# oswsnqc/Tensorflow-DPPO

Measured on AMD Instinct MI355X. Metric: env-steps/sec (whole node), Humanoid-shaped MLP DPPO at 1/2/4/8 MI355X, higher is better.
Workload: dtype fp32; 1 GPU; model=Humanoid-v4 MLP 64x64 tanh, preset=humanoid, global_batch=16777216, num_envs_per_gpu=262144, rollout_T=64, update_steps=4, parallelism=dp1

## Files before the change

dppo_amd/ops/hip/bindings.cpp:

```cpp
#include <torch/extension.h>

#include <vector>

std::vector<torch::Tensor> gae_scan(torch::Tensor rewards, torch::Tensor values,
                                    torch::Tensor dones, torch::Tensor boot,
                                    double gamma, double lam, bool whiten,
                                    double eps, torch::Tensor adv_out,
                                    torch::Tensor etr_out);

torch::Tensor ppo_loss_gauss_fwd(torch::Tensor pdpi, torch::Tensor pdold,
                                 torch::Tensor vpred, torch::Tensor oldv,
                                 torch::Tensor act, torch::Tensor adv,
                                 torch::Tensor etr, double clip,
                                 double entcoeff, double vcoeff);

torch::Tensor ppo_loss_gauss_gh(torch::Tensor pdflat, torch::Tensor oldflat,
                                torch::Tensor vpred, torch::Tensor oldv,
                                torch::Tensor act, torch::Tensor adv,
                                torch::Tensor etr, double clip,
                                double entcoeff, double vcoeff,
                                torch::Tensor clip_dev);

std::vector<torch::Tensor> ppo_loss_gauss_bwd(
    torch::Tensor pdpi, torch::Tensor pdold, torch::Tensor vpred,
    torch::Tensor oldv, torch::Tensor act, torch::Tensor adv,
    torch::Tensor etr, double clip, double entcoeff, double vcoeff,
    torch::Tensor gtotal);

torch::Tensor ppo_loss_cat_fwd(torch::Tensor lpi, torch::Tensor lold,
                               torch::Tensor vpred, torch::Tensor oldv,
                               torch::Tensor act, torch::Tensor adv,
                               torch::Tensor etr, double clip,
                               double entcoeff, double vcoeff);

std::vector<torch::Tensor> ppo_loss_cat_bwd(
    torch::Tensor lpi, torch::Tensor lold, torch::Tensor vpred,
    torch::Tensor oldv, torch::Tensor act, torch::Tensor adv,
    torch::Tensor etr, double clip, double entcoeff, double vcoeff,
    torch::Tensor gtotal);

torch::Tensor cat_sample(torch::Tensor logits, int64_t seed, int64_t ctr);

void bf16_mm256(torch::Tensor A, torch::Tensor B, torch::Tensor C,
                int64_t epi, torch::Tensor bias, torch::Tensor aux,
                torch::Tensor grad, int64_t grad_off, torch::Tensor CT,
                int64_t ldt, torch::Tensor sums, int64_t sums_off);

void bf16_mm_small(torch::Tensor A, torch::Tensor B, torch::Tensor C,
                   torch::Tensor C2, torch::Tensor aux, torch::Tensor grad,
                   int64_t g1_off, int64_t g2_off, int64_t srow, int64_t epi,
                   int64_t m_real, int64_t n_real, int64_t ldc,
                   torch::Tensor bias);

void bf16_transpose(torch::Tensor in, torch::Tensor out, torch::Tensor sums,
                    int64_t sums_off, int64_t R, int64_t C, int64_t ld_in,
                    int64_t ld_out);

void gauss_gh_wide(torch::Tensor pdflat_bf, torch::Tensor oldflat,
                   torch::Tensor v_bf, torch::Tensor oldv, torch::Tensor act,
                   torch::Tensor adv, torch::Tensor etr, torch::Tensor gh,
                   torch::Tensor clip_dev, double clip, double entcoeff,
                   double vcoeff);

void adam_step(torch::Tensor p, torch::Tensor g, torch::Tensor m,
               torch::Tensor v, int64_t step, double lr, double beta1,
               double beta2, double eps);

void adam_step_dev(torch::Tensor p, torch::Tensor g, torch::Tensor m,
                   torch::Tensor v, torch::Tensor step_dev,
                   torch::Tensor lr_dev, torch::Tensor coef, double beta1,
                   double beta2, double eps);

void gemm_fwd(torch::Tensor X, torch::Tensor Wt, torch::Tensor bias,
              int64_t activation, int64_t heads, torch::Tensor C,
              torch::Tensor v, torch::Tensor aux, int64_t wt_layout,
              int64_t ablate, int64_t ldc);

void dw_mfma(torch::Tensor delta, torch::Tensor acts, torch::Tensor grad_buf,
             int64_t w_off, int64_t b_off, int64_t split_row, int64_t w_off2,
             int64_t b_off2, int64_t ablate);

void rollout_sample(torch::Tensor pdflat, torch::Tensor actions,
                    torch::Tensor xva, torch::Tensor seed_dev,
                    torch::Tensor eps_dev, int64_t step, int64_t va_off,
                    double act_low, double act_high);

void gemm_env_step(torch::Tensor xva, torch::Tensor M, torch::Tensor xin,
                   torch::Tensor xout, torch::Tensor envd,
                   torch::Tensor horizons, torch::Tensor t,
                   torch::Tensor epr,
                   torch::Tensor rewards, torch::Tensor dones,
                   torch::Tensor rsum, torch::Tensor seed_dev, double sigma,
                   int64_t step, torch::Tensor V, torch::Tensor xvp);

void rollout_env_step(torch::Tensor xin, torch::Tensor xout, torch::Tensor G,
                      torch::Tensor envd, torch::Tensor horizons,
                      torch::Tensor t, torch::Tensor epr,
                      torch::Tensor rewards, torch::Tensor dones,
                      torch::Tensor seed_dev, double sigma, int64_t step);

torch::Tensor rollout_moments(torch::Tensor rewards, torch::Tensor dones,
                              torch::Tensor epr_in, int64_t T, int64_t E);

bool mlp_chunk_supported(int64_t D, int64_t H, int64_t A, int64_t n_hidden);

void mlp_chunk_train(
    torch::Tensor params, torch::Tensor states, torch::Tensor actions,
    torch::Tensor adv, torch::Tensor etr, torch::Tensor oldflat,
    torch::Tensor oldv, std::vector<int64_t> offsets,
    std::vector<int64_t> dims, int64_t activation, torch::Tensor clip_dev,
    double clip, double entcoeff, double vcoeff, torch::Tensor slabs,
    torch::Tensor mom, torch::Tensor vel, torch::Tensor step_dev,
    torch::Tensor lr_dev, torch::Tensor coef, torch::Tensor flat_grad,
    bool fuse_adam, double beta1, double beta2, double eps);

bool mlp_mid_supported(int64_t H1, int64_t H2, int64_t A, int64_t n_hidden);

void mlp_mid_bwd(torch::Tensor params, std::vector<int64_t> offsets,
                 torch::Tensor h1, torch::Tensor h2, torch::Tensor pdflat,
                 torch::Tensor v, torch::Tensor oldflat, torch::Tensor oldv,
                 torch::Tensor act, torch::Tensor adv, torch::Tensor etr,
                 int64_t activation, torch::Tensor clip_dev, double clip,
                 double entcoeff, double vcoeff, torch::Tensor dz1,
                 torch::Tensor grad);

std::vector<torch::Tensor> rollout_run(
    torch::Tensor params, std::vector<int64_t> offsets,
    std::vector<int64_t> dims, int64_t activation,
    torch::Tensor envblob, int64_t rank, torch::Tensor horizons,
// ... 4 lines not shown

std::vector<torch::Tensor> rollout_run_cat(
    torch::Tensor params, std::vector<int64_t> offsets,
    std::vector<int64_t> dims, int64_t activation,
    torch::Tensor envblob, int64_t rank, torch::Tensor horizons,
    double noise, double eps_explore,
    torch::Tensor x, torch::Tensor t, torch::Tensor epr,
    int64_t T, int64_t n_actions, int64_t seed, torch::Tensor out_buf,
    int64_t ablate);

PYBIND11_MODULE(TORCH_EXTENSION_NAME, mod) {
  mod.def("gae_scan", &gae_scan,
          "segmented GAE reverse scan + whitening (gfx950)");
  mod.def("ppo_loss_gauss_fwd", &ppo_loss_gauss_fwd,
          "fused DiagGaussian PPO loss forward (gfx950)");
  mod.def("ppo_loss_gauss_bwd", &ppo_loss_gauss_bwd,
          "fused DiagGaussian PPO loss backward (gfx950)");
  mod.def("ppo_loss_cat_fwd", &ppo_loss_cat_fwd,
          "fused Categorical PPO loss forward (gfx950)");
  mod.def("ppo_loss_cat_bwd", &ppo_loss_cat_bwd,
          "fused Categorical PPO loss backward (gfx950)");
  mod.def("cat_sample", &cat_sample,
          "Gumbel-max categorical sampling, counter-based RNG (gfx950)");
  mod.def("bf16_mm256", &bf16_mm256,
          "bf16 MFMA GEMM, 256^2 tile, pipelined glds, fused epilogues "
          "(gfx950)");
  mod.def("bf16_mm_small", &bf16_mm_small,
          "guarded bf16 MFMA GEMM for ragged heads shapes (gfx950)");
  mod.def("bf16_transpose", &bf16_transpose,
          "bf16 2D transpose with fused column sums (gfx950)");
  mod.def("gauss_gh_wide", &gauss_gh_wide,
          "wide-policy PPO loss gradient -> bf16 [g_pd | g_v] (gfx950)");
  mod.def("adam_step", &adam_step, "fused flat Adam step (gfx950)");
  mod.def("adam_step_dev", &adam_step_dev,
          "graph-replayable fused Adam (device step/lr) (gfx950)");
  mod.def("rollout_run", &rollout_run,
          "fused T-step rollout: MLP fwd + sample + synthetic env (gfx950)");
  mod.def("rollout_run_cat", &rollout_run_cat,
          "fused T-step rollout, Discrete/Categorical policy: MLP fwd + "
          "Gumbel-max sample + synthetic env, int64 actions (gfx950)");
  mod.def("rollout_sample", &rollout_sample,
          "per-step action sampling + eps-greedy (v3 rollout) (gfx950)");
  mod.def("gemm_env_step", &gemm_env_step,
          "fused G-GEMM + env transition epilogue + per-env finish, "
          "optionally folding the next step's x@V (v3 rollout; gfx950)");
  mod.def("rollout_env_step", &rollout_env_step,
          "per-step synthetic env finish: tanh/reward/done/reset (gfx950)");
  mod.def("rollout_moments", &rollout_moments,
          "episode-reward moments from reward/done streams (gfx950)");
  mod.def("ppo_loss_gauss_gh", &ppo_loss_gauss_gh,
          "wave-per-row PPO loss gradient -> [g_pd | g_v] (gfx950)");
  mod.def("gemm_fwd", &gemm_fwd,
          "MFMA f32 layer forward C=act(X@Wt+b), fused tanh (gfx950)");
  mod.def("dw_mfma", &dw_mfma,
          "MFMA f32 split-K dW += delta^T@acts into flat grad (gfx950)");
  mod.def("mlp_chunk_supported", &mlp_chunk_supported,
          "shape eligibility for the fused chunk-step kernel (gfx950)");
  mod.def("mlp_chunk_train", &mlp_chunk_train,
          "fused small-MLP training chunk step: fwd+PPO grad+bwd+dW "
          "partials + slab-reduce Adam (gfx950)");
  mod.def("mlp_mid_supported", &mlp_mid_supported,
          "shape eligibility for the fused update-middle kernel (gfx950)");
  mod.def("mlp_mid_bwd", &mlp_mid_bwd,
          "fused update middle: PPO grad + heads/L2 dgrad + dW2/heads dW "
          "partials -> dz1 and flat grad, no gh/dz2 in HBM (gfx950)");
}
```

dppo_amd/ops/hip/mfma_gemm.hip:

```cpp

#include <hip/hip_runtime.h>
#include <torch/extension.h>
#include <c10/hip/HIPStream.h>

#include "common.h"

namespace {

using f32x16 = __attribute__((ext_vector_type(16))) float;
using f32x4 = __attribute__((ext_vector_type(4))) float;

constexpr int BK = 16;
constexpr int M_WAVE = 32;
constexpr int FWD_WAVES = 4;
constexpr int FWD_M = FWD_WAVES * M_WAVE;
constexpr int MAX_NT = 4;

DEV_INLINE int cd_row(int reg, int lane) {
  return (reg & 3) + 8 * (reg >> 2) + 4 * (lane >> 5);
}


struct FwdArgs {
  const float* X;
// ... 300 lines not shown
        issue_w(kb + PBK);
      }
      __syncthreads();

      const int ksteps = min(PBK, a.K - kb);
      #pragma unroll 4
      for (int k2 = 0; k2 < ksteps; k2 += 2) {
        const float av = xs[wave * M_WAVE + i_l][k2 + k_l];
        #pragma unroll
        for (int t = 0; t < NT; ++t) {
          const float bv = ws[k2 + k_l][t * M_WAVE + i_l];
          acc[t] = __builtin_amdgcn_mfma_f32_32x32x2f32(av, bv, acc[t], 0, 0, 0);
        }
      }
      __syncthreads();
    }

    #pragma unroll
    for (int t = 0; t < NT; ++t) {
      const int col = n0 + t * M_WAVE + i_l;
      if (col < a.N) {
        const float bv = (a.activation >= 3) ? 0.f : a.bias[col];
        #pragma unroll
        for (int r = 0; r < 16; ++r) {
          const int64_t row = b0 + wave * M_WAVE + cd_row(r, lane);
          if (row < a.B) {
            float x;
            if (a.activation >= 3) {
              const float h = a.aux[row * a.N + col];
              x = acc[t][r] * ((a.activation == 3) ? (1.f - h * h)
                                                   : (h > 0.f ? 1.f : 0.f));
            } else {
              x = acc[t][r] + bv;
              if (a.activation == 0) x = fmaxf(x, 0.f);
              else if (a.activation == 1) x = fast_tanhf(x);
            }
            if (a.heads == 2) {
              if (col == a.N - 2) a.v[row] = x;
              else if (col < a.N - 2) a.C[row * a.ldc + col] = x;
            } else if (a.heads) {
              if (col == a.N - 1) a.v[row] = x;
              else a.C[row * a.ldc + col] = x;
            } else {
              a.C[row * a.ldc + col] = x;
            }
          }
        }
      }
    }
  }
}


template <int RING,
          bool ENV = false>
__launch_bounds__(FWD_WAVES * 64, RING == 2 ? 6 : RING == 3 ? 4 : 3)
__global__ void gemm_fwd_glds_kernel(FwdArgs a) {
  constexpr int NT = 2;
  constexpr int PBK = 16;
  constexpr int NW = NT * M_WAVE;
  constexpr int XB = FWD_M * PBK * 4;
  constexpr int WB = PBK * NW * 4;
  constexpr int SLOT = XB + WB;
  __shared__ __attribute__((aligned(16))) char smem[RING * SLOT];
  const int tid = threadIdx.x;
  const int lane = tid & (WAVE - 1);
  const int wave = tid / WAVE;
  const int i_l = lane & 31;
  const int k_l = lane >> 5;
  const int n0 = blockIdx.y * NW;

  const int64_t b0 = (int64_t)blockIdx.x * FWD_M;
  if (b0 >= a.B) return;

  const float* srcX[2];
  int xcol[2];
  int64_t xrow[2];
  #pragma unroll
  for (int p = 0; p < 2; ++p) {
    const int q = tid + p * FWD_WAVES * 64;
    const int r = q >> 2;
    const int c4 = (q & 3) ^ (r & 3);
    int64_t row = b0 + r;
    row = row < a.B ? row : a.B - 1;
    xrow[p] = row;
    xcol[p] = c4 * 4;
    srcX[p] = a.X + row * a.K;
  }
  const int wk = tid / (NW / 4);
  int wc4 = (tid % (NW / 4)) * 4;
  {
    int c = n0 + wc4;
    c = c + 3 < a.N ? c : a.N - 4;
    wc4 = c;
  }

  const int S_ = (a.K + PBK - 1) / PBK;
  const int phase = (int)(blockIdx.x % (unsigned)S_);
  auto smap = [&](int s) {
    const int t = s + phase;
    return t >= S_ ? t - S_ : t;
  };
  auto issue = [&](int s) {
    const int kb = smap(s) * PBK;
    char* slot = smem + (s % RING) * SLOT;
    #pragma unroll
    for (int p = 0; p < 2; ++p) {
      int col = kb + xcol[p];
      col = col + 3 < a.K ? col : a.K - 4;
      __builtin_amdgcn_global_load_lds(
          (const __attribute__((address_space(1))) unsigned*)(srcX[p] + col),
          (unsigned*)(slot + p * 4096 + wave * 1024), 16, 0, 0);
    }
    int krow = kb + wk;
    krow = krow < a.K ? krow : a.K - 1;
    __builtin_amdgcn_global_load_lds(
        (const __attribute__((address_space(1))) unsigned*)(
            a.Wt + (int64_t)krow * a.N + wc4),
        (unsigned*)(slot + XB + wave * 1024), 16, 0, 0);
  };

  const int S = (a.K + PBK - 1) / PBK;
  #pragma unroll
  for (int p = 0; p < RING - 1; ++p)
    if (p < S) issue(p);

  f32x16 acc[NT];
  #pragma unroll
  for (int t = 0; t < NT; ++t)
    #pragma unroll
    for (int r = 0; r < 16; ++r) acc[t][r] = 0.f;

  for (int s = 0; s < S; ++s) {
    const int rem = min(S - 1 - s, RING - 2);
    if (rem >= RING - 2)
      asm volatile("s_waitcnt vmcnt(%0)" ::"i"(3 * (RING - 2)) : "memory");
    else if (RING == 4 && rem == 1)
      asm volatile("s_waitcnt vmcnt(3)" ::: "memory");
    else
      asm volatile("s_waitcnt vmcnt(0)" ::: "memory");
    __builtin_amdgcn_s_barrier();
    char* slot = smem + (s % RING) * SLOT;
    float* xs = (float*)slot;
    float* ws = (float*)(slot + XB);
    const int kb = smap(s) * PBK;
    if (kb + PBK > a.K) {
      for (int idx = tid; idx < (kb + PBK - a.K) * NW; idx += FWD_WAVES * 64)
        ws[(a.K - kb) * NW + idx] = 0.f;
      __builtin_amdgcn_s_barrier();
    }
    if (s + RING - 1 < S) issue(s + RING - 1);
    #pragma unroll 4
    for (int k2 = 0; k2 < PBK; k2 += 2) {
      const int k = k2 + k_l;
      const int row = wave * M_WAVE + i_l;
      const float av = xs[row * PBK + (((k >> 2) ^ (row & 3)) << 2) + (k & 3)];
      #pragma unroll
      for (int t = 0; t < NT; ++t) {
        const float bv = ws[k * NW + t * M_WAVE + i_l];
        acc[t] = __builtin_amdgcn_mfma_f32_32x32x2f32(av, bv, acc[t], 0, 0, 0);
      }
    }
  }
  asm volatile("s_waitcnt vmcnt(0)" ::: "memory");
  __builtin_amdgcn_s_barrier();

  if constexpr (ENV) {
    constexpr int HR = 16;
    static_assert(RING * SLOT >= FWD_WAVES * HR * NW * 4 + NW * 16 * 4,
                  "env epilogue image + V panel must fit the ring");
    float* tile = reinterpret_cast<float*>(smem) + wave * (HR * NW);
    float* vs = reinterpret_cast<float*>(smem) + FWD_WAVES * HR * NW;
    const bool fold = a.env_xvp != nullptr;
    if (fold) {
      const int kl = tid >> 2;
      const int kr = n0 + kl;
      float4 vv = make_float4(0.f, 0.f, 0.f, 0.f);
      if (kr < a.N)
        vv = *reinterpret_cast<const float4*>(
            &a.env_V[(int64_t)kr * 16 + 4 * (tid & 3)]);
      *reinterpret_cast<float4*>(
          &vs[(kl ^ ((kl >> 2) & 1)) * 16 + 4 * (tid & 3)]) = vv;
      __syncthreads();
    }
    const unsigned seed = (unsigned)(*a.seed_dev);
    const float sigma = a.sigma;
    const int step = a.step;
    const int c4 = lane & 15;
    const int rsub = lane >> 4;
    const int d = n0 + 4 * c4;
    const int c = d >> 2;
    const bool cok = d < a.N;
    float4 dv = make_float4(0.f, 0.f, 0.f, 0.f);
    if (cok) dv = *reinterpret_cast<const float4*>(&a.envd[d]);
    #pragma unroll
    for (int h = 0; h < 2; ++h) {
      int ln = lane;
      asm volatile("" : "+v"(ln));
      #pragma unroll
      for (int t = 0; t < NT; ++t) {
        #pragma unroll
        for (int q = 0; q < 8; ++q) {
          const int lr = cd_row(8 * h + q, ln) - HR * h;
          const int cc = t * M_WAVE + (ln & 31);
          tile[lr * NW + ((((cc >> 2) ^ lr) << 2) | (cc & 3))] =
              acc[t][8 * h + q];
        }
      }
      asm volatile("s_waitcnt lgkmcnt(0)" ::: "memory");
      #pragma unroll
      for (int j = 0; j < 4; ++j) {
        const int lr = 4 * j + rsub;
        const int64_t e = b0 + wave * M_WAVE + HR * h + lr;
        const bool rok = e < a.B;
        float4* slot =
            reinterpret_cast<float4*>(&tile[lr * NW + ((c4 ^ lr) << 2)]);
        float4 v = make_float4(0.f, 0.f, 0.f, 0.f);
        float ss = 0.f;
// ... 19 lines not shown
            v.y = 0.1f * g_rng_normal(seed, (int)e, step, 5000 + d + 1);
            v.z = 0.1f * g_rng_normal(seed, (int)e, step, 5000 + d + 2);
            v.w = 0.1f * g_rng_normal(seed, (int)e, step, 5000 + d + 3);
          }
          *reinterpret_cast<float4*>(&a.env_x[e * a.N + d]) = v;
        }
        #pragma unroll
        for (int off = 8; off > 0; off >>= 1) ss += __shfl_xor(ss, off, 16);
        if (c4 == 0 && rok) a.env_rsum[(int64_t)blockIdx.y * a.B + e] = ss;
        if (fold) *slot = v;
      }
      if (fold) {
        asm volatile("s_waitcnt lgkmcnt(0)" ::: "memory");
        const int fi = lane & 15;
        f32x4 xa = {0.f, 0.f, 0.f, 0.f};
        #pragma unroll
        for (int q = 0; q < 4; ++q) {
          const float4 av = *reinterpret_cast<const float4*>(
              &tile[fi * NW + (((4 * q + rsub) ^ fi) << 2)]);
          const float am[4] = {av.x, av.y, av.z, av.w};
          #pragma unroll
          for (int m = 0; m < 4; ++m) {
            const int k = 4 * (4 * q + rsub) + m;
            const float bv = vs[(k ^ ((k >> 2) & 1)) * 16 + fi];
            xa = __builtin_amdgcn_mfma_f32_16x16x4f32(am[m], bv, xa, 0, 0, 0);
          }
        }
        #pragma unroll
        for (int r = 0; r < 4; ++r) {
          const int64_t e = b0 + wave * M_WAVE + HR * h + 4 * rsub + r;
          if (e < a.B)
            a.env_xvp[((int64_t)blockIdx.y * a.B + e) * 16 + fi] = xa[r];
        }
      }
    }
    return;
  }

  #pragma unroll
  for (int t = 0; t < NT; ++t) {
    const int col = n0 + t * M_WAVE + i_l;
    if (col < a.N) {
      const float bv = (a.activation >= 3) ? 0.f : a.bias[col];
      #pragma unroll
      for (int r = 0; r < 16; ++r) {
        const int64_t row = b0 + wave * M_WAVE + cd_row(r, lane);
        if (row < a.B) {
          float x;
          if (a.activation >= 3) {
            const float h = a.aux[row * a.N + col];
            x = acc[t][r] * ((a.activation == 3) ? (1.f - h * h)
                                                 : (h > 0.f ? 1.f : 0.f));
          } else {
            x = acc[t][r] + bv;
            if (a.activation == 0) x = fmaxf(x, 0.f);
            else if (a.activation == 1) x = fast_tanhf(x);
          }
          if (a.heads == 2) {
            if (col == a.N - 2) a.v[row] = x;
            else if (col < a.N - 2) a.C[row * a.ldc + col] = x;
          } else if (a.heads) {
            if (col == a.N - 1) a.v[row] = x;
            else a.C[row * a.ldc + col] = x;
          } else {
            a.C[row * a.ldc + col] = x;
          }
        }
      }
    }
  }
}

__global__ void env_finish2_kernel(const float* __restrict__ rsum,
                                   int* __restrict__ t,
                                   const int* __restrict__ horizons,
                                   float* __restrict__ epr,
                                   float* __restrict__ rewards,
                                   float* __restrict__ dones, int64_t E,
                                   int D, int npanels) {
  for (int64_t e = gidx(); e < E; e += gstride()) {
    float ss = 0.f;
    for (int p = 0; p < npanels; ++p) ss += rsum[(int64_t)p * E + e];
    const float r = 1.0f - ss / (float)D;
    rewards[e] = r;
    float ep = epr[e] + r;
    int tc = t[e] + 1;
    const int done = tc >= horizons[e] ? 1 : 0;
    dones[e] = (float)done;
    if (done) {
      ep = 0.f;
      tc = 0;
    }
    epr[e] = ep;
    t[e] = tc;
  }
}

__global__ void env_xv_reduce_kernel(const float* __restrict__ xvp,
                                     float* __restrict__ xva, int64_t E,
                                     int kw, int npanels) {
  for (int64_t i = gidx(); i < E * 4; i += gstride()) {
    const int64_t e = i >> 2;
    const int q = (int)(i & 3);
    float4 s = make_float4(0.f, 0.f, 0.f, 0.f);
    for (int p = 0; p < npanels; ++p) {
      const float4 v = *reinterpret_cast<const float4*>(
          &xvp[((int64_t)p * E + e) * 16 + 4 * q]);
      s.x += v.x; s.y += v.y; s.z += v.z; s.w += v.w;
    }
    *reinterpret_cast<float4*>(&xva[e * kw + 4 * q]) = s;
  }
}


struct DwArgs {
  const float* delta;
  const float* acts;
  float* slab;
  float* db_slab;
  int64_t B;
// ... 381 lines not shown
    return e ? atoi(e) : 0;
  }();
  const bool pipe = pipe_env && !a.ablate && K >= 4 &&
                    (K % 4 == 0 || (wt_layout == 0 && activation >= 3)) &&
                    (wt_layout == 1 || (N >= 4 && N % 4 == 0));
  const int pbk = pbk_env ? pbk_env : 16;
  static const int glds_env = []() {
    const char* e = getenv("DPPO_GEMM_GLDS");
    return e ? atoi(e) : 1;
  }();
  const bool glds_ok = glds_env && !a.ablate && wt_layout == 0 &&
                       K % 4 == 0 && K >= 4 && N % 4 == 0 && N >= 4 &&
                       a.activation != 9999;
  const int ring_sel = fwd_ring_for(a.K);
  #define DISPATCH_FWD(NTV, NPANEL)                                          \
    if (glds_ok && NTV == 2 && ring_sel == 2)                                \
      hipLaunchKernelGGL(gemm_fwd_glds_kernel<2>,                            \
                         dim3((unsigned)grid_pipe, NPANEL),                  \
                         dim3(FWD_WAVES * 64), 0, stream, a);                \
    else if (glds_ok && NTV == 2 && ring_sel == 4)                           \
      hipLaunchKernelGGL(gemm_fwd_glds_kernel<4>,                            \
                         dim3((unsigned)grid_pipe, NPANEL),                  \
                         dim3(FWD_WAVES * 64), 0, stream, a);                \
    else if (glds_ok && NTV == 2)                                            \
      hipLaunchKernelGGL(gemm_fwd_glds_kernel<3>,                            \
                         dim3((unsigned)grid_pipe, NPANEL),                  \
                         dim3(FWD_WAVES * 64), 0, stream, a);                \
    else if (pipe && pbk == 32)                                              \
      hipLaunchKernelGGL((gemm_fwd_pipe_kernel<NTV, 32>),                    \
                         dim3(grid_pipe, NPANEL), dim3(FWD_WAVES * 64), 0,   \
                         stream, a);                                         \
    else if (pipe)                                                           \
      hipLaunchKernelGGL((gemm_fwd_pipe_kernel<NTV, 16>),                    \
                         dim3(grid_pipe, NPANEL), dim3(FWD_WAVES * 64), 0,   \
                         stream, a);                                         \
    else                                                                     \
      hipLaunchKernelGGL(gemm_fwd_kernel<NTV>, dim3(grid),                   \
                         dim3(FWD_WAVES * 64), 0, stream, a)
  if (N > MAX_NT * M_WAVE) {
    TORCH_CHECK(pipe, "N > 128 needs the pipelined path (K%4==0 etc.)");
    const int panels = (N + 2 * M_WAVE - 1) / (2 * M_WAVE);
    DISPATCH_FWD(2, panels);
  } else {
    switch (NT) {
      case 1: DISPATCH_FWD(1, 1); break;
      case 2: DISPATCH_FWD(2, 1); break;
      case 3: DISPATCH_FWD(3, 1); break;
      default: DISPATCH_FWD(4, 1); break;
    }
  }
  #undef DISPATCH_FWD
}

void gemm_env_step(torch::Tensor xva, torch::Tensor M, torch::Tensor xin,
                   torch::Tensor xout, torch::Tensor envd,
                   torch::Tensor horizons, torch::Tensor t,
                   torch::Tensor epr,
                   torch::Tensor rewards, torch::Tensor dones,
                   torch::Tensor rsum, torch::Tensor seed_dev, double sigma,
                   int64_t step, torch::Tensor V, torch::Tensor xvp) {
  const int64_t E = xva.size(0);
  const int K = static_cast<int>(xva.size(1));
  const int D = static_cast<int>(M.size(1));
  TORCH_CHECK(xva.is_contiguous() && M.is_contiguous() &&
              xin.is_contiguous() && xout.is_contiguous());
  TORCH_CHECK(M.size(0) == K && xin.size(0) == E && xin.size(1) == D);
  TORCH_CHECK(xout.numel() == E * D);
  TORCH_CHECK(K % 4 == 0 && D % 4 == 0, "fused env step needs 16B rows");
  TORCH_CHECK(horizons.dtype() == torch::kInt32 && t.dtype() == torch::kInt32);
  const int panels_chk = (D + 63) / 64;
  TORCH_CHECK(rsum.numel() >= panels_chk * E);
  FwdArgs a{};
  a.X = xva.data_ptr<float>();
  a.Wt = M.data_ptr<float>();
  a.B = E;
  a.K = K;
  a.N = D;
  a.activation = 5;
  a.ldc = D;
  a.env_xin = xin.data_ptr<float>();
  a.env_x = xout.data_ptr<float>();
  a.envd = envd.data_ptr<float>();
  a.horizons = horizons.data_ptr<int>();
  a.tcount = t.data_ptr<int>();
  a.seed_dev = reinterpret_cast<const long long*>(seed_dev.data_ptr<int64_t>());
  a.env_rsum = rsum.data_ptr<float>();
  a.sigma = (float)sigma;
  a.step = (int)step;
  const int panels = (D + 63) / 64;
  const bool fold = xvp.numel() > 0;
  if (fold) {
    TORCH_CHECK(V.is_contiguous() && V.dim() == 2 && V.size(0) == D &&
                    V.size(1) == 16,
                "x@V fold needs V = [D][16]");
    TORCH_CHECK(K >= 16 && xvp.is_contiguous() &&
                xvp.numel() >= (int64_t)panels * E * 16);
    a.env_V = V.data_ptr<float>();
    a.env_xvp = xvp.data_ptr<float>();
  }
  hipStream_t stream = c10::hip::getCurrentHIPStream().stream();
  const int64_t tiles = (E + FWD_M - 1) / FWD_M;
  const dim3 grid((unsigned)tiles, (unsigned)panels);
  switch (fwd_ring_for(K)) {
    case 2:
      hipLaunchKernelGGL((gemm_fwd_glds_kernel<2, true>), grid,
                         dim3(FWD_WAVES * 64), 0, stream, a);
// ... 148 lines not shown
```

dppo_amd/trainer.py:

```python

from __future__ import annotations

import contextlib
import math
import os
from dataclasses import dataclass
from typing import Dict, Optional, Tuple

import torch

from .config import DPPOConfig, game_spaces
from .envs.synthetic import BatchedSyntheticEnv, make_env
from .models.mlp import PolicyValueMLP
from .ops import gae_advantages, ppo_losses, PPOLossCoeffs
from .parallel.comm import Comm, FlatBuffers
from .utils.logging import ScalarLogger
from .utils.timers import PhaseTimers
from . import spaces

STATS_DIM = 11


@dataclass
class RolloutBatch:
# ... 397 lines not shown
        return self._wt

    def _v3_buffers(self):
        c, env = self.cfg, self.env
        E, T = c.NUM_ENVS, c.MAX_EPOCH_STEPS
        D = self.obs_space.shape[0]
        A = self.act_space.shape[0]
        P = 2 * A
        H = tuple(c.HIDDEN_SIZES)
        key = (E, T, D, A, H)
        if getattr(self, "_v3_key", None) == key:
            return self._v3
        dev = self.device
        r = env.rank_eff
        kw = ((r + A + 3) // 4) * 4
        M = torch.zeros(kw, D, device=dev)
        M[:r] = env.U
        M[r:r + A] = env.B
        B = int(E) * T
        self._v3 = dict(
            xva=torch.zeros(E, kw, device=dev), va_off=r, kw=kw,
            M=M.contiguous(), V=env.V.contiguous(),
            G=torch.empty(E, D, device=dev),
            h=[torch.empty(E, hh, device=dev) for hh in H],
            bz_r=torch.zeros(r, device=dev),
            bz_D=torch.zeros(D, device=dev),
            wh=torch.empty(P + 1, H[-1], device=dev),
            bh=torch.empty(P + 1, device=dev),
            whT_pad=(torch.zeros(H[-1], P + 2, device=dev)
                     if (P + 2) % 4 == 0
                     and os.environ.get("DPPO_HEADS_PAD") != "0" else None),
            bh_pad=torch.zeros(P + 2, device=dev),
            pd_scratch=torch.empty(E, P, device=dev),
            seed_dev=torch.zeros(1, dtype=torch.int64, device=dev),
            eps_dev=torch.zeros(1, dtype=torch.float32, device=dev),
            epr_before=torch.empty(E, device=dev),
            rsum=torch.zeros(((D + 63) // 64) * E, device=dev),
            xvp=(torch.empty(((D + 63) // 64) * E * 16, device=dev)
                 if r == 16 else None),
            empty=torch.empty(0, device=dev),
            acts=torch.empty(sum(B * hh for hh in H), device=dev),
        )
        self._v3_key = key
        return self._v3

    @staticmethod
    def _env_fused() -> bool:
        return os.environ.get("DPPO_ENV_FUSED", "1") != "0"

    @staticmethod
    def _xv_fold() -> bool:
        return os.environ.get("DPPO_XV_FOLD", "0") == "1"

    def _v3_body(self, states, pdflats, actions, values, rewards, dones,
                 boot_v):
        from .ops import hip_ext

        ext = hip_ext()
        c, env, v3 = self.cfg, self.env, self._v3
        E, T = c.NUM_ENVS, c.MAX_EPOCH_STEPS
        D = self.obs_space.shape[0]
        A = self.act_space.shape[0]
        P = 2 * A
        act_code = 1 if c.ACTIVATION == "tanh" else 0
        low = float(self.act_space.low.flat[0])
        high = float(self.act_space.high.flat[0])
        n_h = len(c.HIDDEN_SIZES)
        wh, bh = v3["wh"], v3["bh"]
        wh[:P].copy_(self.pi.pi.weight.detach())
        wh[P:].copy_(self.pi.vf.weight.detach())
        bh[:P].copy_(self.pi.pi.bias.detach())
        bh[P:].copy_(self.pi.vf.bias.detach())
        whT_pad = v3.get("whT_pad")
        if whT_pad is not None:
            whT_pad[:, :P + 1].copy_(wh.t())
            v3["bh_pad"][:P + 1].copy_(bh)
        wts = self._wt_bufs()
        for l, lay in enumerate(self.pi.hidden):
            wts[l].copy_(lay.weight.detach().t())
        v3["epr_before"].copy_(self.epr)
        states[0].reshape(-1).copy_(env.x.reshape(-1))
        hs = c.HIDDEN_SIZES
        B = T * E
        acts_views, off = [], 0
        for hh in hs:
            acts_views.append(v3["acts"].narrow(0, off, B * hh).view(B, hh))
            off += B * hh
        fused = self._env_fused()
        fold = fused and self._xv_fold() and v3["xvp"] is not None
        no_fold = (v3["empty"], v3["empty"])
        for st in range(T):
            xin = states[st]
            h = xin
            for l in range(n_h):
                hl = acts_views[l].narrow(0, st * E, E)
                ext.gemm_fwd(h, wts[l],
                             self.pi.hidden[l].bias.detach(), act_code, 0,
                             hl, hl, hl, 0, 0, 0)
                h = hl
            if whT_pad is not None:
                ext.gemm_fwd(h, whT_pad, v3["bh_pad"], 2, 2, pdflats[st],
                             values[st], pdflats[st], 0, 0, 0)
            else:
                ext.gemm_fwd(h, wh, bh, 2, 1, pdflats[st], values[st],
                             pdflats[st], 1, 0, 0)
            if not fold or st == 0:
                ext.gemm_fwd(xin, v3["V"], v3["bz_r"], 2, 0, v3["xva"],
                             v3["xva"], v3["xva"], 0, 0, v3["kw"])
            ext.rollout_sample(pdflats[st], actions[st], v3["xva"],
                               v3["seed_dev"], v3["eps_dev"], st,
                               v3["va_off"], low, high)
            xout = states[st + 1] if st + 1 < T else env.x
            if fused:
                ext.gemm_env_step(v3["xva"], v3["M"], xin, xout, env.d,
                                  env.horizons_i32, env.t, self.epr,
                                  rewards[st], dones[st], v3["rsum"],
                                  v3["seed_dev"], float(env.NOISE), st,
                                  *((v3["V"], v3["xvp"]) if fold
                                    else no_fold))
            else:
                ext.gemm_fwd(v3["xva"], v3["M"], v3["bz_D"], 2, 0, v3["G"],
                             v3["G"], v3["G"], 0, 0, 0)
                ext.rollout_env_step(xin, xout, v3["G"], env.d,
                                     env.horizons_i32, env.t, self.epr,
                                     rewards[st], dones[st], v3["seed_dev"],
                                     float(env.NOISE), st)
        h = env.x
        for l in range(n_h):
            hl = v3["h"][l]
            ext.gemm_fwd(h, wts[l],
                         self.pi.hidden[l].bias.detach(), act_code, 0,
                         hl, hl, hl, 0, 0, 0)
            h = hl
        if whT_pad is not None:
            ext.gemm_fwd(h, whT_pad, v3["bh_pad"], 2, 2, v3["pd_scratch"],
                         boot_v, v3["pd_scratch"], 0, 0, 0)
        else:
            ext.gemm_fwd(h, wh, bh, 2, 1, v3["pd_scratch"], boot_v,
                         v3["pd_scratch"], 1, 0, 0)
        return ext.rollout_moments(rewards, dones, v3["epr_before"], T, E)

    @torch.no_grad()
    def _rollout_once_hip_v3(self) -> Tuple[RolloutBatch, Dict[str, float]]:
        c, E = self.cfg, self.cfg.NUM_ENVS
        T = c.MAX_EPOCH_STEPS
        eps = self.exploration_rate()
        env = self.env
        self._rollout_counter = getattr(self, "_rollout_counter", 0) + 1
        seed = (
            c.SEED * 1_000_003
            + self.comm.rank * 7_919
            + self._rollout_counter * 104_729
        ) & 0x7FFFFFFFFFFFFFFF
        A = self.act_space.shape[0]
        D = self.obs_space.shape[0]
        P = 2 * A
        n_out = T * E * (D + 3 * A + 3) + E + 5
        if getattr(self, "_rollout_out", None) is None or                 self._rollout_out.numel() != n_out:
            self._rollout_out = torch.empty(n_out, device=self.device)
            self._adv_buf = torch.empty(T * E, device=self.device)
            self._etr_buf = torch.empty(T * E, device=self.device)
        out = self._rollout_out
        o = 0

        def take(shape):
            nonlocal o
            n = 1
            for sd in shape:
                n *= sd
            v = out.narrow(0, o, n).view(shape)
            o += n
            return v

        states = take((T, E, D))
        pdflats = take((T, E, P))
        actions = take((T, E, A))
        values = take((T, E))
        rewards = take((T, E))
        dones = take((T, E))
        boot_v = take((E,))
        v3 = self._v3_buffers()
        v3["seed_dev"].fill_(seed & 0xFFFFFFFF)
        v3["eps_dev"].fill_(float(eps))
        args = (states, pdflats, actions, values, rewards, dones, boot_v)
# ... 641 lines not shown
                batch.oldflat, batch.oldv, batch.actions,
                batch.adv, batch.etr, 0.0,
            )
            self.comm.allreduce_mean_(self.flat_pi.flat_grad)
            self.optimizer.step_captured()

    def _recorded_acts(self, batch: RolloutBatch):
        v3 = self._v3
        B = batch.states.shape[0]
        acts = v3["acts"]
        a_views, off = [], 0
        for hh in self.cfg.HIDDEN_SIZES:
            a_views.append(acts.narrow(0, off, B * hh).view(B, hh))
            off += B * hh
        if self._mid_fused_mode():
            self._Wh_pad = None
            return acts, a_views, batch.oldv, batch.oldflat
        with torch.no_grad():
            Wh_cat = torch.cat(
                [self.pi.pi.weight, self.pi.vf.weight], dim=0).contiguous()
            ldp = (Wh_cat.shape[0] + 3) & ~3
            Wh_pad = torch.zeros(ldp, Wh_cat.shape[1], device=self.device)
            Wh_pad[:Wh_cat.shape[0]] = Wh_cat
            self._Wh_pad = Wh_pad
        return acts, a_views, batch.oldv, batch.oldflat

    def _fused_forward(self, states: torch.Tensor):
        from .ops import hip_ext

        ext = hip_ext()
        c = self.cfg
        B = states.shape[0]
        dims = [self.obs_space.shape[0], *c.HIDDEN_SIZES]
        n_hidden = len(c.HIDDEN_SIZES)
        act_code = 1 if c.ACTIVATION == "tanh" else 0
        with torch.no_grad():
            bs = [lay.bias.detach() for lay in self.pi.hidden]
            wts = self._wt_bufs()
            for l, lay in enumerate(self.pi.hidden):
                wts[l].copy_(lay.weight.detach().t())
            Wh_cat = torch.cat(
                [self.pi.pi.weight, self.pi.vf.weight], dim=0
            ).contiguous()
            Wh_pad = None
            if not self._mid_fused_mode():
                ldp = (Wh_cat.shape[0] + 3) & ~3
                Wh_pad = torch.zeros(ldp, Wh_cat.shape[1],
                                     device=Wh_cat.device)
                Wh_pad[:Wh_cat.shape[0]] = Wh_cat
            bh = torch.cat([self.pi.pi.bias, self.pi.vf.bias]).contiguous()
        total = sum(B * dims[l + 1] for l in range(n_hidden))
        acts = torch.empty(total, device=states.device, dtype=states.dtype)
        a_views, o = [], 0
        x = states
        for l in range(n_hidden):
            n = B * dims[l + 1]
            cview = acts.narrow(0, o, n).view(B, dims[l + 1])
            ext.gemm_fwd(x, wts[l], bs[l],
                         act_code, 0, cview, cview, cview, 0, 0, 0)
            x = cview
            a_views.append(cview)
            o += n
        P = 2 * self.act_space.shape[0]
        pdflat = torch.empty(B, P, device=states.device, dtype=states.dtype)
        v = torch.empty(B, device=states.device, dtype=states.dtype)
        if (P + 2) % 4 == 0 and os.environ.get("DPPO_HEADS_PAD") != "0":
            WhT_pad = torch.zeros(Wh_cat.shape[1], P + 2,
                                  device=states.device)
            WhT_pad[:, :P + 1] = Wh_cat.t()
            bh2 = torch.zeros(P + 2, device=states.device)
            bh2[:P + 1] = bh
            ext.gemm_fwd(x, WhT_pad, bh2, 2, 2, pdflat, v, pdflat, 0, 0, 0)
        else:
            ext.gemm_fwd(x, Wh_cat, bh, 2, 1, pdflat, v, pdflat, 1, 0, 0)
        self._Wh_pad = Wh_pad
        return acts, a_views, v, pdflat

    MID_FUSED_DEFAULT = "load"

    def _mid_fused_mode(self) -> str:
        env = os.environ.get("DPPO_MID_FUSED", self.MID_FUSED_DEFAULT)
        cached = getattr(self, "_mid_mode_cache", None)
        if cached is not None and cached[0] == env:
            return cached[1]
        mode = self._resolve_mid_mode(env)
        self._mid_mode_cache = (env, mode)
        return mode

    def _resolve_mid_mode(self, mode: str) -> str:
        from .ops import hip_ext

        if mode == "0":
            return ""
        if mode != "load":
            raise ValueError(
                f"DPPO_MID_FUSED={mode!r}: expected '0' or 'load'")
        c = self.cfg
        if self._act_kind != "box" or c.DTYPE != "float32":
            return ""
        if c.ACTIVATION not in ("tanh", "relu"):
            return ""
        hs = tuple(c.HIDDEN_SIZES)
        if len(hs) != 2 or not hip_ext().mlp_mid_supported(
                hs[0], hs[1], self.act_space.shape[0], len(hs)):
            return ""
        return mode

    def _mid_backward(self, states, a_views, v, pdflat, oldflat, oldv,
                      actions, adv, etr, clip: float) -> torch.Tensor:
        from .ops import hip_ext

        ext = hip_ext()
        c = self.cfg
        offsets = [sl.start for sl in self.flat_pi.slices]
        grad = self.flat_pi.flat_grad
        dz1 = torch.empty_like(a_views[0])
        ext.mlp_mid_bwd(
            self.flat_pi.flat_param.detach(), offsets, a_views[0], a_views[1],
# ... 183 lines not shown
```

Measured before the change: 108.4 million env-steps/s.

## Fuse policy MLP forward layers, heads and action sampling into one kernel

Adds a fused forward kernel that runs layer 1 through the shared-memory ring mainloop, then holds each wave's 32-row activation tile in LDS to compute layer 2 and the policy/value heads without re-reading h1/h2 from global memory. During rollout it also folds in action sampling, which removes the separate rollout_sample launch. The same kernel is used for the bootstrap value pass and the update forward. This cuts three or four launches per step down to one and drops the intermediate HBM round-trips. The cost is that weights for layers 2 and the heads are read per lane straight from global or cache rather than staged, and occupancy is capped at 4 blocks per CU.

```diff
diff --git a/dppo_amd/ops/hip/bindings.cpp b/dppo_amd/ops/hip/bindings.cpp
--- a/dppo_amd/ops/hip/bindings.cpp
+++ b/dppo_amd/ops/hip/bindings.cpp
@@ -75,6 +75,16 @@
               int64_t activation, int64_t heads, torch::Tensor C,
               torch::Tensor v, torch::Tensor aux, int64_t wt_layout,
               int64_t ablate, int64_t ldc);
+
+bool mlp_fwd_fused_supported(int64_t D, int64_t H1, int64_t H2, int64_t A);
+
+void mlp_fwd_fused(torch::Tensor X, torch::Tensor W1t, torch::Tensor b1,
+                   torch::Tensor W2t, torch::Tensor b2, torch::Tensor WhT_pad,
+                   torch::Tensor bh_pad, int64_t act_code, torch::Tensor h1,
+                   torch::Tensor h2, torch::Tensor pdflat, torch::Tensor v,
+                   torch::Tensor actions, torch::Tensor xva,
+                   torch::Tensor seed_dev, torch::Tensor eps_dev, int64_t step,
+                   int64_t va_off, double act_low, double act_high);
 
 void dw_mfma(torch::Tensor delta, torch::Tensor acts, torch::Tensor grad_buf,
              int64_t w_off, int64_t b_off, int64_t split_row, int64_t w_off2,
@@ -185,6 +195,11 @@
           "wave-per-row PPO loss gradient -> [g_pd | g_v] (gfx950)");
   mod.def("gemm_fwd", &gemm_fwd,
           "MFMA f32 layer forward C=act(X@Wt+b), fused tanh (gfx950)");
+  mod.def("mlp_fwd_fused_supported", &mlp_fwd_fused_supported,
+          "shape eligibility for the fused policy forward (gfx950)");
+  mod.def("mlp_fwd_fused", &mlp_fwd_fused,
+          "fused policy forward: L1 + L2 + heads (+ action sampling) in one "
+          "launch, h1/h2 written once and never re-read (gfx950)");
   mod.def("dw_mfma", &dw_mfma,
           "MFMA f32 split-K dW += delta^T@acts into flat grad (gfx950)");
   mod.def("mlp_chunk_supported", &mlp_chunk_supported,
diff --git a/dppo_amd/ops/hip/mfma_gemm.hip b/dppo_amd/ops/hip/mfma_gemm.hip
--- a/dppo_amd/ops/hip/mfma_gemm.hip
+++ b/dppo_amd/ops/hip/mfma_gemm.hip
@@ -376,26 +376,26 @@
 }
 
 
-template <int RING,
-          bool ENV = false>
-__launch_bounds__(FWD_WAVES * 64, RING == 2 ? 6 : RING == 3 ? 4 : 3)
-__global__ void gemm_fwd_glds_kernel(FwdArgs a) {
-  constexpr int NT = 2;
-  constexpr int PBK = 16;
-  constexpr int NW = NT * M_WAVE;
-  constexpr int XB = FWD_M * PBK * 4;
-  constexpr int WB = PBK * NW * 4;
-  constexpr int SLOT = XB + WB;
-  __shared__ __attribute__((aligned(16))) char smem[RING * SLOT];
+constexpr int GLDS_NT = 2;
+constexpr int GLDS_BK = 16;
+constexpr int GLDS_NW = GLDS_NT * M_WAVE;
+constexpr int GLDS_XB = FWD_M * GLDS_BK * 4;
+constexpr int GLDS_WB = GLDS_BK * GLDS_NW * 4;
+constexpr int GLDS_SLOT = GLDS_XB + GLDS_WB;
+
+template <int RING>
+DEV_INLINE void glds_fwd_mainloop(const FwdArgs& a, char* smem, int64_t b0,
+                                  int n0, f32x16 (&acc)[GLDS_NT]) {
+  constexpr int NT = GLDS_NT;
+  constexpr int PBK = GLDS_BK;
+  constexpr int NW = GLDS_NW;
+  constexpr int XB = GLDS_XB;
+  constexpr int SLOT = GLDS_SLOT;
   const int tid = threadIdx.x;
   const int lane = tid & (WAVE - 1);
   const int wave = tid / WAVE;
   const int i_l = lane & 31;
   const int k_l = lane >> 5;
-  const int n0 = blockIdx.y * NW;
-
-  const int64_t b0 = (int64_t)blockIdx.x * FWD_M;
-  if (b0 >= a.B) return;
 
   const float* srcX[2];
   int xcol[2];
@@ -449,7 +449,6 @@
   for (int p = 0; p < RING - 1; ++p)
     if (p < S) issue(p);
 
-  f32x16 acc[NT];
   #pragma unroll
   for (int t = 0; t < NT; ++t)
     #pragma unroll
@@ -488,6 +487,47 @@
   }
   asm volatile("s_waitcnt vmcnt(0)" ::: "memory");
   __builtin_amdgcn_s_barrier();
+}
+
+DEV_INLINE float fwd_bias_act(float acc, float bv, int activation) {
+  float x = acc + bv;
+  if (activation == 0) x = fmaxf(x, 0.f);
+  else if (activation == 1) x = fast_tanhf(x);
+  return x;
+}
+
+DEV_INLINE void fwd_store(float* C, float* v, int heads, int N, int ldc,
+                          int64_t row, int col, float x) {
+  if (heads == 2) {
+    if (col == N - 2) v[row] = x;
+    else if (col < N - 2) C[row * ldc + col] = x;
+  } else if (heads) {
+    if (col == N - 1) v[row] = x;
+    else C[row * ldc + col] = x;
+  } else {
+    C[row * ldc + col] = x;
+  }
+}
+
+template <int RING,
+          bool ENV = false>
+__launch_bounds__(FWD_WAVES * 64, RING == 2 ? 6 : RING == 3 ? 4 : 3)
+__global__ void gemm_fwd_glds_kernel(FwdArgs a) {
+  constexpr int NT = GLDS_NT;
+  constexpr int NW = GLDS_NW;
+  constexpr int SLOT = GLDS_SLOT;
+  __shared__ __attribute__((aligned(16))) char smem[RING * SLOT];
+  const int tid = threadIdx.x;
+  const int lane = tid & (WAVE - 1);
+  const int wave = tid / WAVE;
+  const int i_l = lane & 31;
+  const int n0 = blockIdx.y * NW;
+
+  const int64_t b0 = (int64_t)blockIdx.x * FWD_M;
+  if (b0 >= a.B) return;
+
+  f32x16 acc[NT];
+  glds_fwd_mainloop<RING>(a, smem, b0, n0, acc);
 
   if constexpr (ENV) {
     constexpr int HR = 16;
@@ -613,20 +653,160 @@
             x = acc[t][r] * ((a.activation == 3) ? (1.f - h * h)
                                                  : (h > 0.f ? 1.f : 0.f));
           } else {
-            x = acc[t][r] + bv;
-            if (a.activation == 0) x = fmaxf(x, 0.f);
-            else if (a.activation == 1) x = fast_tanhf(x);
+            x = fwd_bias_act(acc[t][r], bv, a.activation);
           }
-          if (a.heads == 2) {
-            if (col == a.N - 2) a.v[row] = x;
-            else if (col < a.N - 2) a.C[row * a.ldc + col] = x;
-          } else if (a.heads) {
-            if (col == a.N - 1) a.v[row] = x;
-            else a.C[row * a.ldc + col] = x;
-          } else {
-            a.C[row * a.ldc + col] = x;
-          }
+          fwd_store(a.C, a.v, a.heads, a.N, a.ldc, row, col, x);
         }
+      }
+    }
+  }
+}
+
+
+constexpr int IMG_LD = 65;
+
+struct MlpFwdArgs {
+  FwdArgs l1;
+  const float* W2t;
+  const float* b2;
+  float* h2;
+  const float* WhT;
+  const float* bh;
+  float* pdflat;
+  float* v;
+  int NH;
+  float* actions;
+  float* xva;
+  const long long* seed_dev;
+  const float* eps_dev;
+  int step, xva_w, va_off;
+  float act_low, act_high;
+};
+
+DEV_INLINE float g_rng_uniform(unsigned seed, int env, int step, int slot) {
+  const unsigned h = g_lowbias32(seed ^ (unsigned)env * 0x9E3779B9U ^
+                                 (unsigned)step * 0x85EBCA6BU ^
+                                 (unsigned)slot * 0xC2B2AE35U);
+  return ((h >> 8) + 1) * (1.0f / 16777217.0f);
+}
+
+DEV_INLINE void img_gemm64(const float* img, const float* __restrict__ W,
+                           int N, int phase, int lane,
+                           f32x16 (&acc)[GLDS_NT]) {
+  const int i_l = lane & 31;
+  const int k_l = lane >> 5;
+  #pragma unroll
+  for (int t = 0; t < GLDS_NT; ++t)
+    #pragma unroll
+    for (int r = 0; r < 16; ++r) acc[t][r] = 0.f;
+  const int c0 = i_l < N ? i_l : N - 1;
+  const int c1 = M_WAVE + i_l < N ? M_WAVE + i_l : N - 1;
+  const bool two = N > M_WAVE;
+  #pragma unroll 1
+  for (int s = 0; s < 4; ++s) {
+    const int kb = ((s + phase) & 3) * GLDS_BK;
+    #pragma unroll
+    for (int k2 = 0; k2 < GLDS_BK; k2 += 2) {
+      const int k = kb + k2 + k_l;
+      const float av = img[i_l * IMG_LD + k];
+      const float b0v = W[k * N + c0];
+      acc[0] = __builtin_amdgcn_mfma_f32_32x32x2f32(av, b0v, acc[0], 0, 0, 0);
+      if (two) {
+        const float b1v = W[k * N + c1];
+        acc[1] =
+            __builtin_amdgcn_mfma_f32_32x32x2f32(av, b1v, acc[1], 0, 0, 0);
+      }
+    }
+  }
+}
+
+DEV_INLINE void hidden_epilogue(const f32x16 (&acc)[GLDS_NT],
+                                const float* __restrict__ bias,
+                                int activation, float* C, float* img,
+                                int64_t row0, int64_t B, int lane) {
+  #pragma unroll
+  for (int t = 0; t < GLDS_NT; ++t) {
+    const int col = t * M_WAVE + (lane & 31);
+    const float bv = bias[col];
+    #pragma unroll
+    for (int r = 0; r < 16; ++r) {
+      const int lr = cd_row(r, lane);
+      const float x = fwd_bias_act(acc[t][r], bv, activation);
+      if (row0 + lr < B) C[(row0 + lr) * GLDS_NW + col] = x;
+      img[lr * IMG_LD + col] = x;
+    }
+  }
+}
+
+template <bool SAMPLE>
+__launch_bounds__(FWD_WAVES * 64, 4)
+__global__ void mlp_fwd_fused_kernel(MlpFwdArgs m) {
+  constexpr int RING = 3;
+  static_assert(RING * GLDS_SLOT >= FWD_WAVES * M_WAVE * IMG_LD * 4,
+                "per-wave images must fit the dead stage ring");
+  __shared__ __attribute__((aligned(16))) char smem[RING * GLDS_SLOT];
+  const int lane = threadIdx.x & (WAVE - 1);
+  const int wave = threadIdx.x / WAVE;
+  const int64_t b0 = (int64_t)blockIdx.x * FWD_M;
+  const int64_t B = m.l1.B;
+  if (b0 >= B) return;
+
+  f32x16 acc[GLDS_NT];
+  glds_fwd_mainloop<RING>(m.l1, smem, b0, 0, acc);
+
+  float* img = reinterpret_cast<float*>(smem) + wave * (M_WAVE * IMG_LD);
+  const int64_t row0 = b0 + wave * M_WAVE;
+  const int act = m.l1.activation;
+  const int phase = (int)(blockIdx.x & 3u);
+  const int hphase = m.NH > M_WAVE ? phase : 0;
+
+  hidden_epilogue(acc, m.l1.bias, act, m.l1.C, img, row0, B, lane);
+  asm volatile("s_waitcnt lgkmcnt(0)" ::: "memory");
+  img_gemm64(img, m.W2t, GLDS_NW, phase, lane, acc);
+  asm volatile("s_waitcnt lgkmcnt(0)" ::: "memory");
+  hidden_epilogue(acc, m.b2, act, m.h2, img, row0, B, lane);
+  asm volatile("s_waitcnt lgkmcnt(0)" ::: "memory");
+  img_gemm64(img, m.WhT, m.NH, hphase, lane, acc);
+  asm volatile("s_waitcnt lgkmcnt(0)" ::: "memory");
+
+  const int NH = m.NH;
+  #pragma unroll
+  for (int t = 0; t < GLDS_NT; ++t) {
+    const int col = t * M_WAVE + (lane & 31);
+    if (col < NH) {
+      const float bv = m.bh[col];
+      #pragma unroll
+      for (int r = 0; r < 16; ++r) {
+        const int lr = cd_row(r, lane);
+        const float x = fwd_bias_act(acc[t][r], bv, 2);
+        if (row0 + lr < B)
+          fwd_store(m.pdflat, m.v, 2, NH, NH - 2, row0 + lr, col, x);
+        if constexpr (SAMPLE) img[lr * IMG_LD + col] = x;
+      }
+    }
+  }
+
+  if constexpr (SAMPLE) {
+    asm volatile("s_waitcnt lgkmcnt(0)" ::: "memory");
+    const unsigned seed = (unsigned)*m.seed_dev;
+    const float eps = *m.eps_dev;
+    const int A = (NH - 2) >> 1;
+    const int step = m.step;
+    for (int idx = lane; idx < M_WAVE * A; idx += WAVE) {
+      const int lr = idx / A;
+      const int j = idx - lr * A;
+      const int64_t e = row0 + lr;
+      if (e < B) {
+        const float mean = img[lr * IMG_LD + j];
+        const float logstd = img[lr * IMG_LD + A + j];
+        float a_ = mean + __expf(logstd) * g_rng_normal(seed, (int)e, step, j);
+        const float u_dec = g_rng_uniform(seed, (int)e, step, 90001);
+        if (u_dec < eps) {
+          const float u = g_rng_uniform(seed, (int)e, step, 90010 + j);
+          a_ = m.act_low + (m.act_high - m.act_low) * u;
+        }
+        m.actions[e * A + j] = a_;
+        m.xva[e * m.xva_w + m.va_off + j] = a_;
       }
     }
   }
@@ -1114,6 +1294,91 @@
   #undef DISPATCH_FWD
 }
 
+bool mlp_fwd_fused_supported(int64_t D, int64_t H1, int64_t H2, int64_t A) {
+  const int64_t NH = 2 * A + 2;
+  return D >= 4 && D % 4 == 0 && H1 == GLDS_NW && H2 == GLDS_NW && A >= 1 &&
+         NH % 4 == 0 && NH <= GLDS_NW;
+}
+
+void mlp_fwd_fused(torch::Tensor X, torch::Tensor W1t, torch::Tensor b1,
+                   torch::Tensor W2t, torch::Tensor b2, torch::Tensor WhT_pad,
+                   torch::Tensor bh_pad, int64_t act_code, torch::Tensor h1,
+                   torch::Tensor h2, torch::Tensor pdflat, torch::Tensor v,
+                   torch::Tensor actions, torch::Tensor xva,
+                   torch::Tensor seed_dev, torch::Tensor eps_dev, int64_t step,
+                   int64_t va_off, double act_low, double act_high) {
+  TORCH_CHECK(X.is_cuda() && X.dim() == 2 && X.scalar_type() == torch::kFloat);
+  const int64_t B = X.size(0);
+  const int64_t D = X.size(1);
+  TORCH_CHECK(B >= 1 && WhT_pad.dim() == 2);
+  const int64_t NH = WhT_pad.size(1);
+  const int64_t A = (NH - 2) / 2;
+  TORCH_CHECK(NH == 2 * A + 2 && mlp_fwd_fused_supported(D, W1t.size(1),
+                                                          W2t.size(1), A),
+              "mlp_fwd_fused: shape not eligible");
+  TORCH_CHECK(act_code == 0 || act_code == 1, "mlp_fwd_fused: tanh or relu");
+  for (const auto& t : {X, W1t, b1, W2t, b2, WhT_pad, bh_pad, h1, h2, pdflat, v})
+    TORCH_CHECK(t.is_cuda() && t.is_contiguous() &&
+                t.scalar_type() == torch::kFloat);
+  TORCH_CHECK(W1t.dim() == 2 && W1t.size(0) == D && W2t.dim() == 2 &&
+              W2t.size(0) == GLDS_NW && WhT_pad.size(0) == GLDS_NW);
+  TORCH_CHECK(b1.numel() == GLDS_NW && b2.numel() == GLDS_NW &&
+              bh_pad.numel() == NH);
+  TORCH_CHECK(h1.numel() == B * GLDS_NW && h2.numel() == B * GLDS_NW &&
+              pdflat.numel() == B * (NH - 2) && v.numel() == B);
+
+  MlpFwdArgs m{};
+  m.l1.X = X.data_ptr<float>();
+  m.l1.Wt = W1t.data_ptr<float>();
+  m.l1.bias = b1.data_ptr<float>();
+  m.l1.C = h1.data_ptr<float>();
+  m.l1.B = B;
+  m.l1.K = static_cast<int>(D);
+  m.l1.N = GLDS_NW;
+  m.l1.activation = static_cast<int>(act_code);
+  m.l1.ldc = GLDS_NW;
+  m.W2t = W2t.data_ptr<float>();
+  m.b2 = b2.data_ptr<float>();
+  m.h2 = h2.data_ptr<float>();
+  m.WhT = WhT_pad.data_ptr<float>();
+  m.bh = bh_pad.data_ptr<float>();
+  m.pdflat = pdflat.data_ptr<float>();
+  m.v = v.data_ptr<float>();
+  m.NH = static_cast<int>(NH);
+  const bool sample = actions.numel() > 0;
+  if (sample) {
+    TORCH_CHECK(actions.is_cuda() && actions.is_contiguous() &&
+                actions.scalar_type() == torch::kFloat &&
+                actions.numel() == B * A);
+    TORCH_CHECK(xva.is_cuda() && xva.is_contiguous() && xva.dim() == 2 &&
+                xva.scalar_type() == torch::kFloat && xva.size(0) == B &&
+                va_off >= 0 && va_off + A <= xva.size(1));
+    TORCH_CHECK(seed_dev.is_cuda() && seed_dev.scalar_type() == torch::kLong &&
+                seed_dev.numel() == 1 && eps_dev.is_cuda() &&
+                eps_dev.scalar_type() == torch::kFloat &&
+                eps_dev.numel() == 1);
+    m.actions = actions.data_ptr<float>();
+    m.xva = xva.data_ptr<float>();
+    m.seed_dev =
+        reinterpret_cast<const long long*>(seed_dev.data_ptr<int64_t>());
+    m.eps_dev = eps_dev.data_ptr<float>();
+    m.step = static_cast<int>(step);
+    m.xva_w = static_cast<int>(xva.size(1));
+    m.va_off = static_cast<int>(va_off);
+    m.act_low = static_cast<float>(act_low);
+    m.act_high = static_cast<float>(act_high);
+  }
+  hipStream_t stream = c10::hip::getCurrentHIPStream().stream();
+  const int64_t tiles = (B + FWD_M - 1) / FWD_M;
+  TORCH_CHECK(tiles <= (1 << 22));
+  if (sample)
+    hipLaunchKernelGGL(mlp_fwd_fused_kernel<true>, dim3((unsigned)tiles),
+                       dim3(FWD_WAVES * 64), 0, stream, m);
+  else
+    hipLaunchKernelGGL(mlp_fwd_fused_kernel<false>, dim3((unsigned)tiles),
+                       dim3(FWD_WAVES * 64), 0, stream, m);
+}
+
 void gemm_env_step(torch::Tensor xva, torch::Tensor M, torch::Tensor xin,
                    torch::Tensor xout, torch::Tensor envd,
                    torch::Tensor horizons, torch::Tensor t,
diff --git a/dppo_amd/trainer.py b/dppo_amd/trainer.py
--- a/dppo_amd/trainer.py
+++ b/dppo_amd/trainer.py
@@ -473,6 +473,44 @@
     def _xv_fold() -> bool:
         return os.environ.get("DPPO_XV_FOLD", "0") == "1"
 
+    FWD_FUSED_DEFAULT = "1"
+
+    def _fwd_fused(self) -> bool:
+        key = tuple(os.environ.get(k) for k in (
+            "DPPO_FWD_FUSED", "DPPO_HEADS_PAD", "DPPO_GEMM_GLDS"))
+        cached = getattr(self, "_fwd_fused_cache", None)
+        if cached is not None and cached[0] == key:
+            return cached[1]
+        on = self._resolve_fwd_fused(
+            key[0] if key[0] is not None else self.FWD_FUSED_DEFAULT)
+        self._fwd_fused_cache = (key, on)
+        return on
+
+    def _resolve_fwd_fused(self, mode: str) -> bool:
+        from .ops import hip_ext
+
+        if mode not in ("0", "1"):
+            raise ValueError(f"DPPO_FWD_FUSED={mode!r}: expected '0' or '1'")
+        if mode == "0":
+            return False
+        c = self.cfg
+        if self._act_kind != "box" or c.DTYPE != "float32":
+            return False
+        if c.ACTIVATION not in ("tanh", "relu"):
+            return False
+        if (os.environ.get("DPPO_HEADS_PAD") == "0"
+                or os.environ.get("DPPO_GEMM_GLDS", "1") == "0"):
+            return False
+        hs = tuple(c.HIDDEN_SIZES)
+        return len(hs) == 2 and bool(hip_ext().mlp_fwd_fused_supported(
+            self.obs_space.shape[0], hs[0], hs[1], self.act_space.shape[0]))
+
+    def _count_fwd_fused(self, use: str) -> None:
+        cnt = getattr(self, "fwd_fused_launches", None)
+        if cnt is None:
+            cnt = self.fwd_fused_launches = {}
+        cnt[use] = cnt.get(use, 0) + 1
+
     def _v3_body(self, states, pdflats, actions, values, rewards, dones,
                  boot_v):
         from .ops import hip_ext
@@ -510,27 +548,38 @@
         fused = self._env_fused()
         fold = fused and self._xv_fold() and v3["xvp"] is not None
         no_fold = (v3["empty"], v3["empty"])
+        fwd_fused = whT_pad is not None and self._fwd_fused()
+        hb = [lay.bias.detach() for lay in self.pi.hidden]
         for st in range(T):
             xin = states[st]
             h = xin
-            for l in range(n_h):
-                hl = acts_views[l].narrow(0, st * E, E)
-                ext.gemm_fwd(h, wts[l],
-                             self.pi.hidden[l].bias.detach(), act_code, 0,
-                             hl, hl, hl, 0, 0, 0)
-                h = hl
-            if whT_pad is not None:
-                ext.gemm_fwd(h, whT_pad, v3["bh_pad"], 2, 2, pdflats[st],
-                             values[st], pdflats[st], 0, 0, 0)
+            if fwd_fused:
+                ext.mlp_fwd_fused(
+                    xin, wts[0], hb[0], wts[1], hb[1], whT_pad, v3["bh_pad"],
+                    act_code, acts_views[0].narrow(0, st * E, E),
+                    acts_views[1].narrow(0, st * E, E), pdflats[st],
+                    values[st], actions[st], v3["xva"], v3["seed_dev"],
+                    v3["eps_dev"], st, v3["va_off"], low, high)
+                self._count_fwd_fused("rollout")
             else:
-                ext.gemm_fwd(h, wh, bh, 2, 1, pdflats[st], values[st],
-                             pdflats[st], 1, 0, 0)
+                for l in range(n_h):
+                    hl = acts_views[l].narrow(0, st * E, E)
+                    ext.gemm_fwd(h, wts[l], hb[l], act_code, 0,
+                                 hl, hl, hl, 0, 0, 0)
+                    h = hl
+                if whT_pad is not None:
+                    ext.gemm_fwd(h, whT_pad, v3["bh_pad"], 2, 2, pdflats[st],
+                                 values[st], pdflats[st], 0, 0, 0)
+                else:
+                    ext.gemm_fwd(h, wh, bh, 2, 1, pdflats[st], values[st],
+                                 pdflats[st], 1, 0, 0)
             if not fold or st == 0:
                 ext.gemm_fwd(xin, v3["V"], v3["bz_r"], 2, 0, v3["xva"],
                              v3["xva"], v3["xva"], 0, 0, v3["kw"])
-            ext.rollout_sample(pdflats[st], actions[st], v3["xva"],
-                               v3["seed_dev"], v3["eps_dev"], st,
-                               v3["va_off"], low, high)
+            if not fwd_fused:
+                ext.rollout_sample(pdflats[st], actions[st], v3["xva"],
+                                   v3["seed_dev"], v3["eps_dev"], st,
+                                   v3["va_off"], low, high)
             xout = states[st + 1] if st + 1 < T else env.x
             if fused:
                 ext.gemm_env_step(v3["xva"], v3["M"], xin, xout, env.d,
@@ -547,10 +596,17 @@
                                      rewards[st], dones[st], v3["seed_dev"],
                                      float(env.NOISE), st)
         h = env.x
+        if fwd_fused:
+            ext.mlp_fwd_fused(
+                h, wts[0], hb[0], wts[1], hb[1], whT_pad, v3["bh_pad"],
+                act_code, v3["h"][0], v3["h"][1], v3["pd_scratch"], boot_v,
+                v3["empty"], v3["empty"], v3["seed_dev"], v3["eps_dev"], 0,
+                0, 0.0, 0.0)
+            self._count_fwd_fused("boot")
+            return ext.rollout_moments(rewards, dones, v3["epr_before"], T, E)
         for l in range(n_h):
             hl = v3["h"][l]
-            ext.gemm_fwd(h, wts[l],
-                         self.pi.hidden[l].bias.detach(), act_code, 0,
+            ext.gemm_fwd(h, wts[l], hb[l], act_code, 0,
                          hl, hl, hl, 0, 0, 0)
             h = hl
         if whT_pad is not None:
@@ -1298,18 +1354,33 @@
         total = sum(B * dims[l + 1] for l in range(n_hidden))
         acts = torch.empty(total, device=states.device, dtype=states.dtype)
         a_views, o = [], 0
-        x = states
         for l in range(n_hidden):
             n = B * dims[l + 1]
-            cview = acts.narrow(0, o, n).view(B, dims[l + 1])
-            ext.gemm_fwd(x, wts[l], bs[l],
-                         act_code, 0, cview, cview, cview, 0, 0, 0)
-            x = cview
-            a_views.append(cview)
+            a_views.append(acts.narrow(0, o, n).view(B, dims[l + 1]))
             o += n
         P = 2 * self.act_space.shape[0]
         pdflat = torch.empty(B, P, device=states.device, dtype=states.dtype)
         v = torch.empty(B, device=states.device, dtype=states.dtype)
+        if self._fwd_fused():
+            with torch.no_grad():
+                WhT_pad = torch.zeros(Wh_cat.shape[1], P + 2,
+                                      device=states.device)
+                WhT_pad[:, :P + 1] = Wh_cat.t()
+                bh2 = torch.zeros(P + 2, device=states.device)
+                bh2[:P + 1] = bh
+            empty = states.new_empty(0)
+            ext.mlp_fwd_fused(states, wts[0], bs[0], wts[1], bs[1], WhT_pad,
+                              bh2, act_code, a_views[0], a_views[1], pdflat,
+                              v, empty, empty, empty, empty, 0, 0, 0.0, 0.0)
+            self._count_fwd_fused("update")
+            self._Wh_pad = Wh_pad
+            return acts, a_views, v, pdflat
+        x = states
+        for l in range(n_hidden):
+            ext.gemm_fwd(x, wts[l], bs[l],
+                         act_code, 0, a_views[l], a_views[l], a_views[l],
+                         0, 0, 0)
+            x = a_views[l]
         if (P + 2) % 4 == 0 and os.environ.get("DPPO_HEADS_PAD") != "0":
             WhT_pad = torch.zeros(Wh_cat.shape[1], P + 2,
                                   device=states.device)
```

Result: faster. 111.3 million env-steps/s, median of 6 (+2.6%).
